# astra-vision/rain-rendering

Hardware: AMD Instinct MI355X
Metric: rainy frames/sec @ 1242x375, 100 mm/hr (higher is better)
Workload: dtype f64 alpha/mask, f32 colour

## Files before the change

__graft_entry__.py:

```python
import importlib
import os
import subprocess
import sys
import tempfile

ROOT = os.path.dirname(os.path.abspath(__file__))
if ROOT not in sys.path:
    sys.path.insert(0, ROOT)

CSRC = os.path.join(ROOT, 'rain-rendering_amd', 'csrc')
HIPCC = os.environ.get('HIPCC', '/opt/rocm/bin/hipcc')
HIP_FLAGS = ['--offload-arch=gfx950', '-O3', '-std=c++17', '-ffp-contract=off', '-fPIC', '-shared',
             '-Wno-unused-value', '-Wno-unused-result']


def _newer(target, sources):
    if not os.path.exists(target):
        return True
    t = os.path.getmtime(target)
    return any(os.path.getmtime(s) > t for s in sources)


def build(force=False):
    hip_src = os.path.join(CSRC, 'rainhip.hip')
    host_src = os.path.join(CSRC, 'rr_host.cpp')
    png_src = os.path.join(CSRC, 'rr_png.cpp')
    hip_dep = [hip_src, host_src, png_src] + sorted(os.path.join(CSRC, f) for f in os.listdir(CSRC) if f.endswith('.h')) + \
              [os.path.join(ROOT, 'include', 'rainhip.h')]
    lib = os.path.join(CSRC, 'librainhip.so')
    if force or _newer(lib, hip_dep):
        inc = ['-I' + os.path.join(ROOT, 'include'), '-I' + CSRC]
        objs = [os.path.join(CSRC, 'rainhip.o')]
        compile_flags = [f for f in HIP_FLAGS if f != '-shared']
        subprocess.check_call([HIPCC] + compile_flags + inc + ['-c', hip_src, '-o', objs[0]])
        for src in (host_src, png_src):
            obj = os.path.join(CSRC, os.path.basename(src)[:-4] + '.o')
            subprocess.check_call(['g++', '-O2', '-std=c++17', '-ffp-contract=off', '-fPIC', '-pthread', '-c'] + inc + [src, '-o', obj])
            objs.append(obj)
        subprocess.check_call([HIPCC, '--offload-arch=gfx950', '-fPIC', '-shared'] + objs + ['-lz', '-lpthread', '-o', lib])
    emu_src = os.path.join(ROOT, 'tests', 'hostemu', 'hostemu.cpp')
    emu = os.path.join(ROOT, 'tests', 'hostemu', 'libhostemu.so')
    if force or _newer(emu, [emu_src] + hip_dep[2:]):
        subprocess.check_call(['g++', '-O2', '-std=c++17', '-ffp-contract=off', '-fPIC', '-shared',
                               '-I' + os.path.join(ROOT, 'include'), '-I' + CSRC, emu_src, '-o', emu])
    noise_src = os.path.join(ROOT, 'tests', 'hostemu', 'noise_emu.cpp')
    noise_lib = os.path.join(ROOT, 'tests', 'hostemu', 'libnoiseemu.so')
    if force or _newer(noise_lib, [noise_src] + hip_dep[3:]):
        subprocess.check_call(['g++', '-O2', '-std=c++17', '-ffp-contract=off', '-fPIC', '-shared',
                               '-I' + os.path.join(ROOT, 'include'), '-I' + CSRC, noise_src, '-o', noise_lib])
    field_src = os.path.join(ROOT, 'tests', 'hostemu', 'field_emu.cpp')
    field_lib = os.path.join(ROOT, 'tests', 'hostemu', 'libfieldemu.so')
    if force or _newer(field_lib, [field_src] + hip_dep[3:]):
        subprocess.check_call(['g++', '-O2', '-std=c++17', '-ffp-contract=off', '-fPIC', '-shared',
                               '-I' + os.path.join(ROOT, 'include'), '-I' + CSRC, field_src, '-o', field_lib])
    rig_src = os.path.join(ROOT, 'tests', 'hostemu', 'rig_emu.cpp')
    rig_lib = os.path.join(ROOT, 'tests', 'hostemu', 'librigemu.so')
    if force or _newer(rig_lib, [rig_src] + hip_dep[3:]):
        subprocess.check_call(['g++', '-O2', '-std=c++17', '-ffp-contract=off', '-fPIC', '-shared',
                               '-I' + os.path.join(ROOT, 'include'), '-I' + CSRC, rig_src, '-o', rig_lib])
    importlib.import_module('rain-rendering_amd')
    hb = importlib.import_module('rain-rendering_amd.hip_backend')
    hb.load_library()


def smoke():
    import numpy as np
    build()
    sys.path.insert(0, os.path.join(ROOT, 'tests'))
    import helpers as h
    with tempfile.TemporaryDirectory() as tmp:
        sc = h.Scene(tmp, 96, 160, 120)
        bg, env = sc.frame_inputs(0)
        drops = sc.product_drops(0)
        rh = h.hb.RainHip(0)
        rh.set_streak_db(sc.db.streaks_light)
        rh.set_camera(sc.cam)
        out = rh.render_frames([dict(bg=bg, rainy_bg=bg, env_xyY=env, omega=sc.omega, drops=drops)])[0]
        ref = h.oracle_render(sc, 0, bg, bg, env, faithful=True)
        assert np.array_equal(out['status'], ref['status']), 'drop status mismatch'
        assert np.array_equal(out['mask'], ref['mask']), 'rainy_mask (f64) not bit-exact'
        assert np.array_equal(out['mask_i32'], ref['mask_i32']), 'rainy_mask (i32) not bit-exact'
        d = np.abs(out['image_u8'].astype(int) - ref['image_u8'].astype(int)).max()
        assert d <= 1, 'rainy_image differs by %d LSB' % d
        rh.close()
    print('smoke ok: %d drops, mask bit-exact, image max |d| = %d LSB' % (len(drops), d))


if __name__ == '__main__':
    build(force='--force' in sys.argv)
    if '--smoke' in sys.argv:
        smoke()
```

rain-rendering_amd/csrc/rainhip.hip:

```cpp
#include <hip/hip_runtime.h>

#include <dlfcn.h>

#include <cstddef>
#include <cstdio>
#include <cstdlib>
#include <algorithm>
#include <cstring>
#include <string>
#include <mutex>
#include <unordered_map>
#include <vector>

#include "rainhip.h"
#include "rr_device.h"
#include "rr_prepass.h"
#include "rr_deflate.h"
#include "rr_pngrows.h"
#include "rr_particles.h"

using namespace rr;

namespace {

// ... 2395 lines not shown
    }
  }
}

__global__ __launch_bounds__(1024) void k_rows_scatter(int max_drops, Scratch sc) {
  const int f = blockIdx.x, t = threadIdx.x;
  __shared__ int s_start[RW_TEX_MAX], s_rank[RW_TEX_MAX];
  const int nf = sc.rows_n[3 * f] + sc.rows_n[3 * f + 1];
  if (nf == 0) return;
  const int own = t < sc.n_buckets ? sc.rows_hist[t] : 0;
  s_start[t] = own;
  __syncthreads();
  for (int ofs = 1; ofs < 1024; ofs <<= 1) {
    const int v = t >= ofs ? s_start[t - ofs] : 0;
    __syncthreads();
    s_start[t] += v;
    __syncthreads();
  }
  const int excl = s_start[t] - own;
  __syncthreads();
  s_start[t] = excl;
  s_rank[t] = t < sc.n_buckets ? sc.rows_fbase[(int64_t)f * RW_TEX_MAX + t] : 0;
  __syncthreads();
  const int64_t base = (int64_t)f * max_drops;
  for (int j = t; j < nf; j += 1024) {
    const int i = sc.rows_list[base + j];
    const DropPlan& p = sc.plan[base + i];
    const int tex = p.tex + (p.kind == KIND_BIG ? sc.n_tex : 0);
    const int pos = s_start[tex] + atomicAdd(&s_rank[tex], 1);
    sc.rows_sorted[pos] = (int32_t)(base + i);
  }
}

__device__ void gauss_half_table(double sigma, int r, double* hw ) {
  const int t = threadIdx.x;
  for (int k = t; k <= r; k += blockDim.x) hw[k] = gauss_phi(sigma, r - k);
  __syncthreads();
  __shared__ double s_tot;
  if (t == 0) {
    double tot = 0.0;
    for (int x = -r; x <= r; x++) tot = tot + hw[r - (x < 0 ? -x : x)];
    s_tot = tot;
  }
  __syncthreads();
  const double tot = s_tot;
  for (int k = t; k <= r; k += blockDim.x) hw[k] = hw[k] / tot;
  __syncthreads();
}


constexpr int BW_LANES = 4;
__global__ __launch_bounds__(256) void k_blur_weights(const FrameDesc* frames, int max_drops, Scratch sc) {
  constexpr int NG = 256 / BW_LANES;
  __shared__ double s_hw[NG][BR_MAX + 2];
  const int f = blockIdx.y, grp = threadIdx.x / BW_LANES, l = threadIdx.x % BW_LANES;
  const int idx = blockIdx.x * NG + grp;
  const int i = idx >> 1, axis = idx & 1;
  int r = 0;
  double sigma = 0.0;
  const int64_t gi = (int64_t)f * max_drops + (i < frames[f].n_drops ? i : 0);
  if (i < frames[f].n_drops) {
    const DropPlan& p = sc.plan[gi];
    if (p.status == RR_DROP_OK && sc.sizes[gi] != 0 && p.r1 > 0 && p.r1 <= BR_MAX) {
      r = axis ? p.r2 : p.r1;
      sigma = axis ? p.sig2 : p.sig1;
    }
  }
  double* tab = s_hw[grp];
  for (int k = l; k <= r && r > 0; k += BW_LANES) tab[k] = gauss_phi(sigma, r - k);
  wave_lds_sync();
  if (l == 0 && r > 0) {
    double tot = 0.0;
    for (int x = -r; x <= r; x++) tot = tot + tab[r - (x < 0 ? -x : x)];
    tab[BR_MAX + 1] = tot;
  }
  wave_lds_sync();
  if (r > 0) {
    const double tot = tab[BR_MAX + 1];
    double* hw = sc.wtab + (gi * 2 + axis) * (BR_MAX + 1);
    for (int k = l; k <= r; k += BW_LANES) hw[k] = tab[k] / tot;
  }
}

template <class W>
__device__ inline void blur4(const double* c0, int st, W hw, int r, double& acc0, double& acc1, double& acc2, double& acc3) {
  auto at = [&](int k) { return c0[__mul24(k, st)]; };
  const double wc = hw(r);
  acc0 = c0[0] * wc; acc1 = at(1) * wc; acc2 = at(2) * wc; acc3 = at(3) * wc;
  double a0 = at(-r), a1 = at(1 - r), a2 = at(2 - r), a3 = at(3 - r);
  double b0 = at(r), b1 = at(1 + r), b2 = at(2 + r), b3 = at(3 + r);
  int ii = -r;
  for (; ii + 3 < 0; ii += 4) {
    const double w0 = hw(ii + r), w1 = hw(ii + 1 + r), w2 = hw(ii + 2 + r), w3 = hw(ii + 3 + r);
    const double na0 = at(4 + ii), na1 = at(5 + ii), na2 = at(6 + ii), na3 = at(7 + ii);
    const double nb0 = at(-ii - 1), nb1 = at(-ii - 2), nb2 = at(-ii - 3), nb3 = at(-ii - 4);
    acc0 = acc0 + (a0 + b0) * w0; acc1 = acc1 + (a1 + b1) * w0; acc2 = acc2 + (a2 + b2) * w0; acc3 = acc3 + (a3 + b3) * w0;
    acc0 = acc0 + (a1 + nb0) * w1; acc1 = acc1 + (a2 + b0) * w1; acc2 = acc2 + (a3 + b1) * w1; acc3 = acc3 + (na0 + b2) * w1;
    acc0 = acc0 + (a2 + nb1) * w2; acc1 = acc1 + (a3 + nb0) * w2; acc2 = acc2 + (na0 + b0) * w2; acc3 = acc3 + (na1 + b1) * w2;
    acc0 = acc0 + (a3 + nb2) * w3; acc1 = acc1 + (na0 + nb1) * w3; acc2 = acc2 + (na1 + nb0) * w3; acc3 = acc3 + (na2 + b0) * w3;
    a0 = na0; a1 = na1; a2 = na2; a3 = na3;
    b3 = nb0; b2 = nb1; b1 = nb2; b0 = nb3;
  }
  for (; ii < 0; ii++) {
    const double w = hw(ii + r);
    const double na = at(4 + ii);
    const double nb = at(-ii - 1);
    acc0 = acc0 + (a0 + b0) * w;
    acc1 = acc1 + (a1 + b1) * w;
    acc2 = acc2 + (a2 + b2) * w;
    acc3 = acc3 + (a3 + b3) * w;
    a0 = a1; a1 = a2; a2 = a3; a3 = na;
    b3 = b2; b2 = b1; b1 = b0; b0 = nb;
  }
}

template <int NO, class W>
__device__ inline void blur_n(const double* c0, int st, W hw, int r, double (&acc)[NO]) {
  const double wc = hw(r);
#pragma unroll
  for (int j = 0; j < NO; j++) acc[j] = c0[__mul24(j, st)] * wc;
  for (int ii = -r; ii < 0; ii++) {
    const double w = hw(ii + r);
#pragma unroll
    for (int j = 0; j < NO; j++) acc[j] = acc[j] + (c0[__mul24(j + ii, st)] + c0[__mul24(j - ii, st)]) * w;
  }
}

__device__ inline void glds_dword(const void* src, uint32_t lds_byte) {
  uint32_t keep;
  asm volatile("s_mov_b32 %0, m0\n\ts_mov_b32 m0, %2\n\ts_nop 0\n\tglobal_load_lds_dword %1, off\n\ts_mov_b32 m0, %0"
               : "=&s"(keep)
               : "v"(src), "s"(__builtin_amdgcn_readfirstlane((int)lds_byte))
               : "memory");
}
__device__ inline void glds_dwordx4(const void* src, uint32_t lds_byte) {
  uint32_t keep;
  asm volatile("s_mov_b32 %0, m0\n\ts_mov_b32 m0, %2\n\ts_nop 0\n\tglobal_load_lds_dwordx4 %1, off\n\ts_mov_b32 m0, %0"
               : "=&s"(keep)
               : "v"(src), "s"(__builtin_amdgcn_readfirstlane((int)lds_byte))
               : "memory");
}
__global__ __launch_bounds__(256, 4) void k_blur_fused_dma(const FrameDesc* frames, int max_drops, Scratch sc) {
  const int f = blockIdx.y, t = threadIdx.x, lane = t & 63, G = gridDim.x;
  const int wave = __builtin_amdgcn_readfirstlane(t >> 6);
  extern __shared__ __attribute__((aligned(16))) double s_dyn[];
  constexpr int TAB = 2 * (BR_MAX + 1);
  double* tabs = s_dyn;
  double* X = s_dyn + 2 * TAB;
  double* Y = X + sc.blur_bx;
  const uint32_t lds_tabs = (uint32_t)(uintptr_t)(__attribute__((address_space(3))) double*)tabs;
  const uint32_t lds_x = (uint32_t)(uintptr_t)(__attribute__((address_space(3))) double*)X;
  const int n_items = sc.counts[f * 8 + 2];
  if ((int)blockIdx.x >= n_items) return;
  const global_ptr<const uint32_t> items_w = as_global(reinterpret_cast<const uint32_t*>(sc.blur_items + (int64_t)f * max_drops * BLUR_ITEMS_PER_DROP));
  const DropPlan* plans = sc.plan + (int64_t)f * max_drops;
  auto load_item = [&](int item) { return items_w[(int64_t)item * 4 + (lane & 3)]; };
  auto load_plan = [&](int i) { return as_global(reinterpret_cast<const uint32_t*>(plans + i))[lane]; };
  struct PlanView {
    int r1, r2, ew, eh, tw, th, epitch, epad;
    long long a0_off, a1_off;
  };
  auto unpack = [&](uint32_t pv) {
    auto F = [&](size_t byte_off) { return (int)__builtin_amdgcn_readlane((int)pv, (int)(byte_off / 4)); };
    PlanView o;
    o.r1 = F(offsetof(DropPlan, r1)); o.r2 = F(offsetof(DropPlan, r2)); o.ew = F(offsetof(DropPlan, ew)); o.eh = F(offsetof(DropPlan, eh));
    o.tw = F(offsetof(DropPlan, tw)); o.th = F(offsetof(DropPlan, th)); o.epitch = F(offsetof(DropPlan, epitch)); o.epad = F(offsetof(DropPlan, epad));
    o.a0_off = (long long)(((unsigned long long)(unsigned)F(offsetof(DropPlan, a0_off) + 4) << 32) | (unsigned)F(offsetof(DropPlan, a0_off)));
    o.a1_off = (long long)(((unsigned long long)(unsigned)F(offsetof(DropPlan, a1_off) + 4) << 32) | (unsigned)F(offsetof(DropPlan, a1_off)));
    return o;
  };
  auto item_of = [&](uint32_t iv) {
    return make_int4((int)__builtin_amdgcn_readlane((int)iv, 0), (int)__builtin_amdgcn_readlane((int)iv, 1),
                     (int)__builtin_amdgcn_readlane((int)iv, 2), (int)__builtin_amdgcn_readlane((int)iv, 3));
  };
  struct Geo {
    int y0, x0, ho, wo, hop, hi, yp, xa, wd, nx, xs, ys, e_lo, e_hi;
  };
  auto geo = [&](const PlanView& p, int Lwo, int Lho, int st) {
    Geo g;
    const int ntx = (p.ew + Lwo - 1) / Lwo;
    const int sty = st / ntx, stx = st - sty * ntx;
    g.y0 = sty * Lho; g.x0 = stx * Lwo;
    g.ho = imin(Lho, p.eh - g.y0);
    g.wo = imin(Lwo, p.ew - g.x0);
    g.hop = (g.ho + 3) & ~3;
    const int wi = g.wo + 2 * p.r2;
    g.hi = g.hop + 2 * p.r1;
    g.yp = blur_y_pitch(g.wo, p.r2);
    g.xa = imax(0, 2 * p.r2 - g.x0);
    const int xb = imin(wi, p.tw + 2 * p.r2 - g.x0);
    g.wd = imax(xb - g.xa, 0);
    g.nx = g.wd * g.hi;
    g.xs = g.x0 - 2 * p.r2 + g.xa; g.ys = g.y0 - 2 * p.r1;
    const int ra = imin(imax(-g.ys, 0), g.hi), rb = imax(imin(p.th - g.ys, g.hi), ra);
    g.e_lo = ra * g.wd; g.e_hi = rb * g.wd;
    return g;
  };
  auto stage = [&](const PlanView& p, const Geo& g, int drop, bool tables, int tb) {
    if (g.e_hi > g.e_lo && g.wd == p.tw) {
      const char* src = reinterpret_cast<const char*>(sc.arena + p.a0_off + (int64_t)g.ys * p.tw);
      const int a = (g.e_lo + 1) & ~1, b = g.e_hi & ~1;
      for (int e0 = (a & ~511); e0 < b; e0 += 512) {
        const int e = e0 + wave * 128 + 2 * lane;
        if (e >= a && e < b) glds_dwordx4(src + (int64_t)e * 8, lds_x + (uint32_t)(e0 + wave * 128) * 8u);
      }
      if (wave == 0 && (g.e_lo & 1) && lane < 2) glds_dword(src + (int64_t)g.e_lo * 8 + lane * 4, lds_x + (uint32_t)g.e_lo * 8u);
      if (wave == 1 && (g.e_hi & 1) && g.e_hi - 1 >= g.e_lo && lane < 2) glds_dword(src + (int64_t)(g.e_hi - 1) * 8 + lane * 4, lds_x + (uint32_t)(g.e_hi - 1) * 8u);
    } else if (g.e_hi > g.e_lo) {
      const int wdd = imax(g.wd, 1);
      const float inv_wd = 1.0f / (float)wdd;
      const int dq = (int)((128.0f + 0.5f) * inv_wd), dr = 128 - dq * wdd;
      const char* src = reinterpret_cast<const char*>(sc.arena + p.a0_off) + (lane & 1) * 4;
      const int c0 = g.e_lo >> 7, c1 = (g.e_hi + 127) >> 7;
      int e = c0 * 128 + wave * 32 + (lane >> 1);
      int yy = (int)(((float)e + 0.5f) * inv_wd), xc = e - yy * wdd;
      for (int c = c0; c < c1; c++) {
        if (e >= g.e_lo && e < g.e_hi)
          glds_dword(src + (int64_t)((g.ys + yy) * p.tw + (g.xs + xc)) * 8, lds_x + (uint32_t)(c * 128 + wave * 32) * 8u);
        e += 128;
        xc += dr;
        yy += dq;
        if (xc >= wdd) { xc -= wdd; yy += 1; }
      }
    }
    if (tables) {
      const char* wt = reinterpret_cast<const char*>(sc.wtab + ((int64_t)f * max_drops + drop) * TAB);
      if (wave == 3 && lane < TAB / 2) glds_dwordx4(wt + lane * 16, lds_tabs + (uint32_t)(tb * TAB) * 8u);
    }
  };
  uint32_t iv0 = load_item(blockIdx.x);
  uint32_t pv0 = load_plan((int)__builtin_amdgcn_readlane((int)iv0, 0));
  uint32_t iv1 = load_item(imin((int)blockIdx.x + G, n_items - 1));
  uint32_t pv1 = load_plan((int)__builtin_amdgcn_readlane((int)iv1, 0));
  uint32_t iv2 = load_item(imin((int)blockIdx.x + 2 * G, n_items - 1));
  int it = blockIdx.x;
  int4 item = item_of(iv0);
  PlanView p = unpack(pv0);
  int st = item.y, tb = 0;
  Geo g = geo(p, item.w & 0xffff, item.w >> 16, st);
  stage(p, g, item.x, true, tb);
  PH_DECL
  for (;;) {
    const int r1 = p.r1, r2 = p.r2;
    const double* hw1 = tabs + tb * TAB;
    const double* hw2 = hw1 + (BR_MAX + 1);
    {
      const int nz2 = (g.yp * g.hop + 1) >> 1;
      double2* Y2 = reinterpret_cast<double2*>(Y);
      for (int i = t; i < nz2; i += 256) Y2[i] = make_double2(0.0, 0.0);
    }
    asm volatile("s_waitcnt vmcnt(0)" ::: "memory");
    bool has_next = true, new_item = false;
    int4 nitem = item;
    PlanView np = p;
    int nst = st + 1, ntb = tb;
    if (nst >= item.y + item.z) {
      if (it + G < n_items) {
        new_item = true;
        nitem = item_of(iv1);
        np = unpack(pv1);
        nst = nitem.y;
        if (nitem.x != item.x) ntb = tb ^ 1;
      } else {
        has_next = false;
      }
    }
    {
      iv1 = new_item ? iv2 : iv1;
      pv1 = load_plan((int)__builtin_amdgcn_readlane((int)iv1, 0));
      iv2 = load_item(imin(new_item ? it + 3 * G : it + 2 * G, n_items - 1));
    }
    for (int i = t; i < g.e_lo; i += 256) X[i] = 0.0;
    for (int i = g.e_hi + t; i < g.nx; i += 256) X[i] = 0.0;
    PH(0)
    __syncthreads();
    PH(1)
    {
      const int wd = g.wd, nrb = g.hop >> 2, nv = nrb * wd;
      const float inv_wd = 1.0f / (float)imax(wd, 1);
      for (int idx = t; idx < nv; idx += 256) {
        const int rb = (int)(((float)idx + 0.5f) * inv_wd), xq = idx - rb * wd;
        const double* c0 = X + (4 * rb + r1) * wd + xq;
        double acc0, acc1, acc2, acc3;
        blur4(c0, wd, [&](int k) { return hw1[k]; }, r1, acc0, acc1, acc2, acc3);
        double* o = Y + 4 * rb * g.yp + g.xa + xq;
        o[0] = acc0;
        o[g.yp] = acc1;
        o[2 * g.yp] = acc2;
        o[3 * g.yp] = acc3;
      }
    }
    PH(2)
    __syncthreads();
    PH(3)
    Geo ng = g;
    if (has_next) {
      ng = geo(np, nitem.w & 0xffff, nitem.w >> 16, nst);
      stage(np, ng, nitem.x, ntb != tb, ntb);
    }
    PH(6)
    {
      const int ncb = (g.wo + 3) >> 2, nh = ncb * g.ho;
      const float inv_ho = 1.0f / (float)g.ho;
      double* dst = sc.arena + p.a1_off;
      for (int idx = t; idx < nh; idx += 256) {
        const int cb = (int)(((float)idx + 0.5f) * inv_ho), yq = idx - cb * g.ho;
        const double* c0 = Y + yq * g.yp + 4 * cb + r2;
        double acc0, acc1, acc2, acc3;
        if (r2 > 0) {
          blur4(c0, 1, [&](int k) { return hw2[k]; }, r2, acc0, acc1, acc2, acc3);
        } else {
          acc0 = c0[0]; acc1 = c0[1]; acc2 = c0[2]; acc3 = c0[3];
        }
        const int xo = 4 * cb;
        double* o = dst + (int64_t)(g.y0 + yq) * p.epitch + p.epad + (g.x0 + xo);
        if (xo + 3 < g.wo) {
          o[0] = acc0; o[1] = acc1; o[2] = acc2; o[3] = acc3;
        } else {
          o[0] = acc0;
          if (xo + 1 < g.wo) o[1] = acc1;
          if (xo + 2 < g.wo) o[2] = acc2;
        }
      }
    }
    PH(4)
    if (!has_next) break;
    __syncthreads();
    PH(5)
    if (new_item) it += G;
    item = nitem; p = np; st = nst; tb = ntb; g = ng;
  }
  PH_FLUSH(3)
}

typedef double double2_v __attribute__((ext_vector_type(2)));
struct SmallItem {
  int li, r1, r2, tw, th, pw, ph, epitch, epad;
  long long a0, a1;
};
__global__ __launch_bounds__(256, 4) void k_blur_small(const FrameDesc* frames, int max_drops, Scratch sc) {
  const int f = blockIdx.y, lane = threadIdx.x & 63, wave = threadIdx.x >> 6;
  __shared__ __attribute__((aligned(16))) double Xs[4][BS_X], Ys[4][BS_Y];
  double* X = Xs[wave];
  double* Y = Ys[wave];
  const int n_items = sc.counts[f * 8 + 4];
  const global_ptr<const int32_t> list = as_global(sc.list_small + (int64_t)f * max_drops);
  const DropPlan* plans = sc.plan + (int64_t)f * max_drops;
  const int stride = gridDim.x * 4;
  int it = blockIdx.x * 4 + wave;
  if (it >= n_items) return;
  auto load_plan = [&](int li) { return as_global(reinterpret_cast<const uint32_t*>(plans + li))[lane]; };
  auto unpack = [&](uint32_t pv, int li) {
    auto F = [&](size_t byte_off) { return (int)__builtin_amdgcn_readlane((int)pv, (int)(byte_off / 4)); };
    static_assert(offsetof(DropPlan, a1_off) + 8 <= 256, "DropPlan layout");
    SmallItem o;
    o.li = li;
    o.r1 = F(offsetof(DropPlan, r1)); o.r2 = F(offsetof(DropPlan, r2)); o.tw = F(offsetof(DropPlan, tw)); o.th = F(offsetof(DropPlan, th));
    o.pw = F(offsetof(DropPlan, ew)); o.ph = F(offsetof(DropPlan, eh)); o.epitch = F(offsetof(DropPlan, epitch)); o.epad = F(offsetof(DropPlan, epad));
    o.a0 = (long long)(((unsigned long long)(unsigned)F(offsetof(DropPlan, a0_off) + 4) << 32) | (unsigned)F(offsetof(DropPlan, a0_off)));
    o.a1 = (long long)(((unsigned long long)(unsigned)F(offsetof(DropPlan, a1_off) + 4) << 32) | (unsigned)F(offsetof(DropPlan, a1_off)));
    return o;
  };
  double2_v R[4];
  double nw1 = 0.0, nw2 = 0.0;
  auto issue = [&](const SmallItem& d) {
    const global_ptr<const double2_v> raw2 = as_global(reinterpret_cast<const double2_v*>(sc.arena + d.a0));
    const int n = d.tw * d.th;
#pragma unroll
    for (int j = 0; j < 4; j++) {
      const int k2 = lane + 64 * j;
      R[j] = double2_v{0.0, 0.0};
      if (2 * k2 < n) R[j] = raw2[k2];
    }
    const global_ptr<const double> wt = as_global(sc.wtab + ((int64_t)f * max_drops + d.li) * 2 * (BR_MAX + 1));
    nw1 = (lane <= d.r1) ? wt[d.r1 - lane] : 0.0;
    nw2 = (d.r2 > 0 && lane <= d.r2) ? wt[(BR_MAX + 1) + d.r2 - lane] : 0.0;
  };
  PH_DECL
  const int li0 = __builtin_amdgcn_readfirstlane(list[it]);
  SmallItem cur = unpack(load_plan(li0), li0);
  issue(cur);
  bool has_next = it + stride < n_items;
  int li1 = has_next ? __builtin_amdgcn_readfirstlane(list[it + stride]) : li0;
  uint32_t pv_next = load_plan(li1);
  int32_t li2_v = (it + 2 * stride < n_items) ? list[it + 2 * stride] : 0;
  for (;;) {
    const int r1 = cur.r1, r2 = cur.r2, pw = cur.pw, ph = cur.ph, tw = cur.tw, th = cur.th;
    const int php = (ph + 3) & ~3, hi = php + 2 * r1, yp = blur_y_pitch(pw, r2);
    double* tile = sc.arena + cur.a1;
    {
      const int n = tw * th, top = 2 * r1 * tw;
      double2* X2 = reinterpret_cast<double2*>(X);
#pragma unroll
      for (int j = 0; j < 4; j++) {
        const int k2 = lane + 64 * j;
        if (2 * k2 < n) X2[(top >> 1) + k2] = make_double2(R[j].x, 2 * k2 + 1 < n ? R[j].y : 0.0);
      }
      for (int i = lane; i < (top >> 1); i += 64) X2[i] = make_double2(0.0, 0.0);
      const int e0 = (top + n + 1) >> 1, e1 = (tw * hi + 1) >> 1;
      for (int i = e0 + lane; i < e1; i += 64) X2[i] = make_double2(0.0, 0.0);
      const int nz2 = (yp * php + 1) >> 1;
      double2* Y2 = reinterpret_cast<double2*>(Y);
      for (int i = lane; i < nz2; i += 64) Y2[i] = make_double2(0.0, 0.0);
    }
    const double w1 = nw1, w2 = nw2;
    wave_lds_sync();
    PH(0)
    SmallItem nxt = cur;
    if (has_next) {
      nxt = unpack(pv_next, li1);
      issue(nxt);
      if (it + 2 * stride < n_items) {
        li1 = __builtin_amdgcn_readfirstlane(li2_v);
        pv_next = load_plan(li1);
        if (it + 3 * stride < n_items) li2_v = list[it + 3 * stride];
      }
    }
    const float inv_tw = 1.0f / (float)tw;
    const int nv4 = (php >> 2) * tw;
    if (nv4 <= 16) {
      const int idx = lane;
      if (idx < 4 * nv4) {
        const int row = (int)(((float)idx + 0.5f) * inv_tw), x = idx - row * tw;
        double a[1];
        blur_n<1>(X + (__mul24(row + r1, tw) + x), tw, [&](int k) { return readlane_f64(w1, r1 - k); }, r1, a);
        Y[__mul24(row, yp) + 2 * r2 + x] = a[0];
      }
    } else if (nv4 <= 32) {
      const int idx = lane;
      if (idx < 2 * nv4) {
        const int rb = (int)(((float)idx + 0.5f) * inv_tw), x = idx - rb * tw;
        double a[2];
        blur_n<2>(X + (__mul24(2 * rb + r1, tw) + x), tw, [&](int k) { return readlane_f64(w1, r1 - k); }, r1, a);
        double* o = Y + (__mul24(2 * rb, yp) + 2 * r2 + x);
        o[0] = a[0];
        o[yp] = a[1];
      }
    } else {
      const int nv = nv4;
      for (int idx = lane; idx < nv; idx += 64) {
        const int rb = (int)(((float)idx + 0.5f) * inv_tw), x = idx - rb * tw;
        const double* c0 = X + (__mul24(4 * rb + r1, tw) + x);
        double a0, a1, a2, a3;
        blur4(c0, tw, [&](int k) { return readlane_f64(w1, r1 - k); }, r1, a0, a1, a2, a3);
        double* o = Y + (__mul24(4 * rb, yp) + 2 * r2 + x);
        o[0] = a0;
        o[yp] = a1;
        o[2 * yp] = a2;
        o[3 * yp] = a3;
      }
    }
    wave_lds_sync();
    PH(1)
    const int ncb = (pw + 3) >> 2, nh = ncb * ph;
    const float inv_ph = 1.0f / (float)ph;
    if (nh <= 16 && r2 > 0) {
      const int idx = lane;
      if (idx < pw * ph) {
        const int x = (int)(((float)idx + 0.5f) * inv_ph), yq = idx - x * ph;
        double a[1];
        blur_n<1>(Y + (__mul24(yq, yp) + x + r2), 1, [&](int k) { return readlane_f64(w2, r2 - k); }, r2, a);
        tile[(int64_t)yq * cur.epitch + cur.epad + x] = a[0];
      }
    } else if (nh <= 32 && r2 > 0) {
      const int idx = lane, nc2 = (pw + 1) >> 1;
      if (idx < nc2 * ph) {
        const int cb = (int)(((float)idx + 0.5f) * inv_ph), yq = idx - cb * ph, xo = 2 * cb;
        double a[2];
        blur_n<2>(Y + (__mul24(yq, yp) + xo + r2), 1, [&](int k) { return readlane_f64(w2, r2 - k); }, r2, a);
        double* o = tile + (int64_t)yq * cur.epitch + cur.epad + xo;
        o[0] = a[0];
        if (xo + 1 < pw) o[1] = a[1];
      }
    } else {
      for (int idx = lane; idx < nh; idx += 64) {
        const int cb = (int)(((float)idx + 0.5f) * inv_ph), yq = idx - cb * ph;
        const double* c0 = Y + (__mul24(yq, yp) + 4 * cb + r2);
        double a0, a1, a2, a3;
        if (r2 > 0) {
          blur4(c0, 1, [&](int k) { return readlane_f64(w2, r2 - k); }, r2, a0, a1, a2, a3);
        } else {
          a0 = c0[0]; a1 = c0[1]; a2 = c0[2]; a3 = c0[3];
        }
        const int xo = 4 * cb;
        double* o = tile + (int64_t)yq * cur.epitch + cur.epad + xo;
        if (xo + 3 < pw) {
          o[0] = a0; o[1] = a1; o[2] = a2; o[3] = a3;
        } else {
          o[0] = a0;
          if (xo + 1 < pw) o[1] = a1;
          if (xo + 2 < pw) o[2] = a2;
        }
      }
    }
    wave_lds_sync();
    PH(2)
    if (!has_next) break;
    it += stride;
    cur = nxt;
    has_next = it + stride < n_items;
  }
  PH_FLUSH(2)
}

constexpr int BIG_GROUPS = 64;
constexpr int BIG_ROWS = 16;
constexpr int BIG_COL_LDS = 2048;

template <class F>
__device__ inline void visit_taps(int a0, int a1, int b0, int b1, int r, F f) {
  a0 = imax(a0, -r); a1 = imin(a1, -1);
  b0 = imax(b0, -r); b1 = imin(b1, -1);
  if (a0 > a1) { a0 = b0; a1 = b1; b0 = 0; b1 = -1; }
  if (b0 <= b1 && b0 < a0) { int t = a0; a0 = b0; b0 = t; t = a1; a1 = b1; b1 = t; }
  if (b0 <= b1 && b0 <= a1 + 1) { a1 = imax(a1, b1); b0 = 0; b1 = -1; }
  for (int ii = a0; ii <= a1; ii++) f(ii);
  for (int ii = b0; ii <= b1; ii++) f(ii);
}

constexpr int SLOW_CAP = 256;
__global__ __launch_bounds__(256) void k_blur_big_weights(const FrameDesc* frames, int max_drops, Scratch sc) {
  const int f = blockIdx.y;
  __shared__ double hw[MAX_R + 1];
  const int n_items = imin(sc.counts[f * 8 + 3], SLOW_CAP);
  for (int w = blockIdx.x; w < 2 * n_items; w += gridDim.x) {
    const int it = w >> 1, axis = w & 1;
    const DropPlan& p = sc.plan[(int64_t)f * max_drops + sc.list_slow[(int64_t)f * max_drops + it]];
    const int r = axis ? p.r2 : p.r1;
    __syncthreads();
    if (r > 0) {
      gauss_half_table(axis ? p.sig2 : p.sig1, r, hw);
      double* o = sc.wtab_big + (((int64_t)f * SLOW_CAP + it) * 2 + axis) * (MAX_R + 1);
      for (int k = threadIdx.x; k <= r; k += 256) o[k] = hw[k];
    }
  }
}

template <int AXIS>
__global__ __launch_bounds__(256) void k_blur(const FrameDesc* frames, int max_drops, Scratch sc) {
  const int f = blockIdx.y, t = threadIdx.x;
  __shared__ double hw[MAX_R + 1];
  __shared__ double s_in[BIG_COL_LDS];
  const int n_items = sc.counts[f * 8 + 3];
  int cur = -1;
  for (int w = blockIdx.x; w < n_items * BIG_GROUPS; w += gridDim.x) {
    const int it = w / BIG_GROUPS, g = w - it * BIG_GROUPS;
    const int64_t gi = (int64_t)f * max_drops + sc.list_slow[(int64_t)f * max_drops + it];
    const DropPlan& p = sc.plan[gi];
    const int r = AXIS == 0 ? p.r1 : p.r2;
    const int tw = p.tw, th = p.th, ew = p.ew, eh = p.eh, r1 = p.r1, r2 = p.r2;
    if (AXIS == 0 ? g >= tw : g * BIG_ROWS >= eh) continue;
    const double* raw = sc.arena + p.a0_off;
    double* fin = sc.arena + p.a1_off;
    double* tmp = fin + (((int64_t)p.epitch * eh + 15) & ~15LL);
    __syncthreads();
    if (cur != it) {
      if (r > 0) {
        if (it < SLOW_CAP) {
          const double* wt = sc.wtab_big + (((int64_t)f * SLOW_CAP + it) * 2 + AXIS) * (MAX_R + 1);
          for (int k = t; k <= r; k += 256) hw[k] = wt[k];
          __syncthreads();
        } else {
          gauss_half_table(AXIS == 0 ? p.sig1 : p.sig2, r, hw);
        }
      }
      cur = it;
    }
    if (AXIS == 0) {
      for (int rx = g; rx < tw; rx += BIG_GROUPS) {
        const bool lds = th <= BIG_COL_LDS;
        __syncthreads();
        if (lds)
          for (int k = t; k < th; k += 256) s_in[k] = raw[(int64_t)k * tw + rx];
        __syncthreads();
// ... 4182 lines not shown
```

rain-rendering_amd/csrc/rr_device.h:

```cpp
#pragma once
#include <math.h>
#include <stdint.h>

#include "rainhip.h"

#if defined(__HIPCC__)
#include <hip/hip_runtime.h>
#define RR_HD __host__ __device__ inline
#else
#define RR_HD inline
#endif

#if defined(__clang__)
#pragma clang fp contract(off)
#endif

namespace rr {

enum { KIND_BIG = 0, KIND_ROT = 1, KIND_EXT = 2 };
enum { RS_AREA = 0, RS_AREA_FAST = 1, RS_LINEAR = 2 };

struct Dims {
  int32_t H, W, He, We;
};
// ... 1230 lines not shown
      else p.rs_mode = RS_AREA;
    } else {
      p.rs_mode = RS_LINEAR;
    }
    minCx = d.x0;
    minCy = d.y0;
  }

  if (strategy == 1) {
    p.pw = p.tw;
    p.ph = p.th;
    const int sx = py_slice_index(minCx, W), ex = py_slice_index(minCx + p.tw, W);
    const int sy = py_slice_index(minCy, H), ey = py_slice_index(minCy + p.th, H);
    p.vis_x0 = sx;
    p.vis_y0 = sy;
    p.vis_w = imax(ex - sx, 0);
    p.vis_h = imax(ey - sy, 0);
    p.tau_one = cam.exposure_s * 1.0;
    p.g = p.tau_one / cam.tau_zero;
    p.ew = p.tw;
    p.eh = p.th;
    size_out = (p.vis_w > 0 && p.vis_h > 0) ? (((int64_t)p.tw * p.th + 15) & ~15LL) : 0;
    return;
  }
  double o = fabs(d.wps[2]);
  double cc = ((o - cam.focus_plane) * cam.focal_sq) / (o * (cam.focus_plane - cam.focal_m) * cam.f_number);
  cc = fabs(cc / cam.sensor_px);
  if (!(cc < 1.7e308)) { p.status = RR_DROP_BAD_COC; return; }
  if (10.0 * cc >= (double)(RR_MAX_SHIFT + 1)) { p.status = RR_DROP_TOO_BIG; return; }
  p.shift = (int)(10.0 * cc);
  p.sig1 = cc;
  p.sig2 = cc / 2.0;
  p.r1 = (p.sig1 > 1e-15) ? (int)(4.0 * p.sig1 + 0.5) : 0;
  p.r2 = (p.sig2 > 1e-15) ? (int)(4.0 * p.sig2 + 0.5) : 0;
  p.pw = p.tw + 2 * p.shift;
  p.ph = p.th + 2 * p.shift;

  int tmpx = minCx - p.shift, tmpy = minCy - p.shift;
  int mcx = imin(imax(tmpx, 0), W), mcy = imin(imax(tmpy, 0), H);
  int dx = mcx - tmpx, dy = mcy - tmpy;
  int cw, ch;
  if (dx < 0) { cw = imax(p.pw + dx, 0); p.crop_x = 0; } else { cw = imax(p.pw - dx, 0); p.crop_x = dx; }
  if (dy < 0) { ch = imax(p.ph + dy, 0); p.crop_y = 0; } else { ch = imax(p.ph - dy, 0); p.crop_y = dy; }
  p.vis_x0 = mcx;
  p.vis_y0 = mcy;
  p.vis_w = imax(imin(mcx + cw, W) - mcx, 0);
  p.vis_h = imax(imin(mcy + ch, H) - mcy, 0);

  double d_avg = (d.iw1 + d.iw2) / 2.0;
  double length_opacity = opacity_attenuation * d_avg / ((double)d.length + d_avg);
  p.tau_one = cam.exposure_s * length_opacity;
  p.g = p.tau_one / cam.tau_zero;

  p.ew = p.tw + 2 * p.r2;
  p.eh = p.th + 2 * p.r1;
  p.epad = 0;
  p.epitch = p.ew;
  size_out = (p.vis_w > 0 && p.vis_h > 0) ? (((int64_t)p.tw * p.th + 15) & ~15LL) + (p.r1 > 0 ? (((int64_t)p.epitch * p.eh + 15) & ~15LL) : 0) : 0;
}

RR_HD double blur_axis0(const double* src, int pw, int ph, int x, int y, const double* hw, int r) {
  double acc = src[(int64_t)y * pw + x] * hw[r];
  for (int ii = -r; ii < 0; ii++) {
    int ya = y + ii, yb = y - ii;
    double va = (ya >= 0) ? src[(int64_t)ya * pw + x] : 0.0;
    double vb = (yb < ph) ? src[(int64_t)yb * pw + x] : 0.0;
    acc = acc + (va + vb) * hw[ii + r];
  }
  return acc;
}
RR_HD double blur_axis1(const double* src, int pw, int ph, int x, int y, const double* hw, int r) {
  (void)ph;
  const double* row = src + (int64_t)y * pw;
  double acc = row[x] * hw[r];
  for (int ii = -r; ii < 0; ii++) {
    int xa = x + ii, xb = x - ii;
    double va = (xa >= 0) ? row[xa] : 0.0;
    double vb = (xb < pw) ? row[xb] : 0.0;
    acc = acc + (va + vb) * hw[ii + r];
  }
  return acc;
}

RR_HD void blend_pixel(double A, double tau_one, double exposure, double g, const double K[3], double bgr[3], double& mask) {
  double t = (A * tau_one) / exposure;
  double u = 1.0 - t;
  for (int c = 0; c < 3; c++) {
    double v = u * bgr[c] + (A * K[c]) * g;
    bgr[c] = clip01(v);
  }
  mask = mask + A;
}

constexpr int BLUR_BX = 2816;
constexpr int BLUR_BY = 2048;
constexpr int BR_MAX = 48;

struct BlurLayout {
  int fused;
  int wo, ho;
  int single;
};
RR_HD int blur_x_doubles(int wo, int ho, int r1, int r2, int tw) { return imin(wo + 2 * r2, tw) * (((ho + 3) & ~3) + 2 * r1); }
RR_HD int blur_y_pitch(int wo, int r2) { return (((wo + 3) & ~3) + 2 * r2) | 1; }
RR_HD int blur_y_doubles(int wo, int ho, int r2) { return blur_y_pitch(wo, r2) * ((ho + 3) & ~3); }

RR_HD BlurLayout blur_layout(const DropPlan& p, int BX_MAX, int BY_MAX) {
  BlurLayout b{0, 0, 0, 0};
  if (p.r1 <= 0 || p.r1 > BR_MAX) return b;
  if (blur_x_doubles(p.ew, p.eh, p.r1, p.r2, p.tw) <= BX_MAX && blur_y_doubles(p.ew, p.eh, p.r2) <= BY_MAX) {
    b.fused = 1; b.wo = p.ew; b.ho = p.eh; b.single = 1;
    return b;
  }
  {
    const int hy = (BY_MAX / blur_y_pitch(p.ew, p.r2)) & ~3;
    const int hx = ((BX_MAX / imin(p.ew + 2 * p.r2, p.tw)) - 2 * p.r1) & ~3;
    const int hb = imin(hy, hx);
    if (hb >= imax(8, p.r1)) {
      b.fused = 1; b.wo = p.ew; b.ho = imin(hb, p.eh);
      return b;
    }
  }
  const double rr2 = (double)imax(p.r2, 1), rr1 = (double)p.r1;
  int wi = (int)sqrt((double)BX_MAX * rr2 / rr1);
  wi = imax(imin(wi, p.ew + 2 * p.r2), 2 * p.r2 + 4);
  int hi = BX_MAX / wi;
  hi = imin(hi, ((p.eh + 3) & ~3) + 2 * p.r1);
  wi = imin(BX_MAX / hi, p.ew + 2 * p.r2);
  int wo = wi - 2 * p.r2, ho = (hi - 2 * p.r1) & ~3;
  if (ho > p.eh) ho = p.eh;
  for (int it = 0; it < 64 && wo >= 1 && ho >= 1; it++) {
    if (blur_x_doubles(wo, ho, p.r1, p.r2, p.tw) <= BX_MAX && blur_y_doubles(wo, ho, p.r2) <= BY_MAX) {
      b.fused = 1; b.wo = wo; b.ho = ho; b.single = (wo >= p.ew && ho >= p.eh) ? 1 : 0;
      return b;
    }
    if (blur_x_doubles(wo, ho, p.r1, p.r2, p.tw) > BX_MAX) { if (wo > 4) wo -= 1; else ho -= 4; }
    else ho -= 4;
  }
  return b;
}
constexpr int BS_X = 512;
constexpr int BS_Y = 768;

RR_HD bool blur_is_small(const DropPlan& p) {
  const int php = (p.eh + 3) & ~3;
  return p.r1 > 0 && p.r1 <= 31 && p.tw * (php + 2 * p.r1) <= BS_X && blur_y_pitch(p.ew, p.r2) * php <= BS_Y;
}


}
```

Measured before the change: 18440.

## Blur eight outputs per thread with a generic sliding-window kernel

Replaces the hand-unrolled 4-output separable blur with a templated sliding-window routine. Larger tiles now process 8 rows or columns per thread, with a 4-wide tail, so each loaded sample is reused across more outputs. The per-item Y buffer clear now zeroes only the padding columns instead of the whole buffer. The change also adds readfirstlane hints for wave-uniform offsets and the wave index, plus a host emulator build for the blur. Register pressure rises with 8 accumulators under launch_bounds(256,4), and any mismatch in the reassociated summation order would break the required bit-exact masks.

```diff
diff --git a/__graft_entry__.py b/__graft_entry__.py
--- a/__graft_entry__.py
+++ b/__graft_entry__.py
@@ -58,6 +58,11 @@
     if force or _newer(rig_lib, [rig_src] + hip_dep[3:]):
         subprocess.check_call(['g++', '-O2', '-std=c++17', '-ffp-contract=off', '-fPIC', '-shared',
                                '-I' + os.path.join(ROOT, 'include'), '-I' + CSRC, rig_src, '-o', rig_lib])
+    blur_src = os.path.join(ROOT, 'tests', 'hostemu', 'blur_emu.cpp')
+    blur_lib = os.path.join(ROOT, 'tests', 'hostemu', 'libbluremu.so')
+    if force or _newer(blur_lib, [blur_src] + hip_dep[3:]):
+        subprocess.check_call(['g++', '-O2', '-std=c++17', '-ffp-contract=off', '-fPIC', '-shared',
+                               '-I' + os.path.join(ROOT, 'include'), '-I' + CSRC, blur_src, '-o', blur_lib])
     importlib.import_module('rain-rendering_amd')
     hb = importlib.import_module('rain-rendering_amd.hip_backend')
     hb.load_library()
diff --git a/rain-rendering_amd/csrc/rainhip.hip b/rain-rendering_amd/csrc/rainhip.hip
--- a/rain-rendering_amd/csrc/rainhip.hip
+++ b/rain-rendering_amd/csrc/rainhip.hip
@@ -2501,49 +2501,6 @@
   }
 }
 
-template <class W>
-__device__ inline void blur4(const double* c0, int st, W hw, int r, double& acc0, double& acc1, double& acc2, double& acc3) {
-  auto at = [&](int k) { return c0[__mul24(k, st)]; };
-  const double wc = hw(r);
-  acc0 = c0[0] * wc; acc1 = at(1) * wc; acc2 = at(2) * wc; acc3 = at(3) * wc;
-  double a0 = at(-r), a1 = at(1 - r), a2 = at(2 - r), a3 = at(3 - r);
-  double b0 = at(r), b1 = at(1 + r), b2 = at(2 + r), b3 = at(3 + r);
-  int ii = -r;
-  for (; ii + 3 < 0; ii += 4) {
-    const double w0 = hw(ii + r), w1 = hw(ii + 1 + r), w2 = hw(ii + 2 + r), w3 = hw(ii + 3 + r);
-    const double na0 = at(4 + ii), na1 = at(5 + ii), na2 = at(6 + ii), na3 = at(7 + ii);
-    const double nb0 = at(-ii - 1), nb1 = at(-ii - 2), nb2 = at(-ii - 3), nb3 = at(-ii - 4);
-    acc0 = acc0 + (a0 + b0) * w0; acc1 = acc1 + (a1 + b1) * w0; acc2 = acc2 + (a2 + b2) * w0; acc3 = acc3 + (a3 + b3) * w0;
-    acc0 = acc0 + (a1 + nb0) * w1; acc1 = acc1 + (a2 + b0) * w1; acc2 = acc2 + (a3 + b1) * w1; acc3 = acc3 + (na0 + b2) * w1;
-    acc0 = acc0 + (a2 + nb1) * w2; acc1 = acc1 + (a3 + nb0) * w2; acc2 = acc2 + (na0 + b0) * w2; acc3 = acc3 + (na1 + b1) * w2;
-    acc0 = acc0 + (a3 + nb2) * w3; acc1 = acc1 + (na0 + nb1) * w3; acc2 = acc2 + (na1 + nb0) * w3; acc3 = acc3 + (na2 + b0) * w3;
-    a0 = na0; a1 = na1; a2 = na2; a3 = na3;
-    b3 = nb0; b2 = nb1; b1 = nb2; b0 = nb3;
-  }
-  for (; ii < 0; ii++) {
-    const double w = hw(ii + r);
-    const double na = at(4 + ii);
-    const double nb = at(-ii - 1);
-    acc0 = acc0 + (a0 + b0) * w;
-    acc1 = acc1 + (a1 + b1) * w;
-    acc2 = acc2 + (a2 + b2) * w;
-    acc3 = acc3 + (a3 + b3) * w;
-    a0 = a1; a1 = a2; a2 = a3; a3 = na;
-    b3 = b2; b2 = b1; b1 = b0; b0 = nb;
-  }
-}
-
-template <int NO, class W>
-__device__ inline void blur_n(const double* c0, int st, W hw, int r, double (&acc)[NO]) {
-  const double wc = hw(r);
-#pragma unroll
-  for (int j = 0; j < NO; j++) acc[j] = c0[__mul24(j, st)] * wc;
-  for (int ii = -r; ii < 0; ii++) {
-    const double w = hw(ii + r);
-#pragma unroll
-    for (int j = 0; j < NO; j++) acc[j] = acc[j] + (c0[__mul24(j + ii, st)] + c0[__mul24(j - ii, st)]) * w;
-  }
-}
 
 __device__ inline void glds_dword(const void* src, uint32_t lds_byte) {
   uint32_t keep;
@@ -2695,18 +2652,35 @@
     __syncthreads();
     PH(1)
     {
-      const int wd = g.wd, nrb = g.hop >> 2, nv = nrb * wd;
+      const int wd = g.wd, nv4 = (g.hop >> 2) * wd;
       const float inv_wd = 1.0f / (float)imax(wd, 1);
-      for (int idx = t; idx < nv; idx += 256) {
-        const int rb = (int)(((float)idx + 0.5f) * inv_wd), xq = idx - rb * wd;
-        const double* c0 = X + (4 * rb + r1) * wd + xq;
-        double acc0, acc1, acc2, acc3;
-        blur4(c0, wd, [&](int k) { return hw1[k]; }, r1, acc0, acc1, acc2, acc3);
-        double* o = Y + 4 * rb * g.yp + g.xa + xq;
-        o[0] = acc0;
-        o[g.yp] = acc1;
-        o[2 * g.yp] = acc2;
-        o[3 * g.yp] = acc3;
+      auto w1 = [&](int k) { return hw1[k]; };
+      auto rows4 = [&](int row, int xq) {
+        double acc[4];
+        blur4(X + (row + r1) * wd + xq, wd, w1, r1, acc);
+        double* o = Y + row * g.yp + g.xa + xq;
+#pragma unroll
+        for (int j = 0; j < 4; j++) o[__mul24(j, g.yp)] = acc[j];
+      };
+      if (nv4 > 256) {
+        const int n8 = (g.hop >> 3) * wd, n4 = (g.hop & 4) ? wd : 0;
+        for (int idx = t; idx < n8 + n4; idx += 256) {
+          if (idx < n8) {
+            const int rb = (int)(((float)idx + 0.5f) * inv_wd), xq = idx - rb * wd;
+            double acc[8];
+            blur8(X + (8 * rb + r1) * wd + xq, wd, w1, r1, acc);
+            double* o = Y + 8 * rb * g.yp + g.xa + xq;
+#pragma unroll
+            for (int j = 0; j < 8; j++) o[__mul24(j, g.yp)] = acc[j];
+          } else {
+            rows4(g.hop & ~7, idx - n8);
+          }
+        }
+      } else {
+        for (int idx = t; idx < nv4; idx += 256) {
+          const int rb = (int)(((float)idx + 0.5f) * inv_wd);
+          rows4(4 * rb, idx - rb * wd);
+        }
       }
     }
     PH(2)
@@ -2719,26 +2693,58 @@
     }
     PH(6)
     {
-      const int ncb = (g.wo + 3) >> 2, nh = ncb * g.ho;
+      const int wop = (g.wo + 3) & ~3, nh4 = (wop >> 2) * g.ho;
       const float inv_ho = 1.0f / (float)g.ho;
       double* dst = sc.arena + p.a1_off;
-      for (int idx = t; idx < nh; idx += 256) {
-        const int cb = (int)(((float)idx + 0.5f) * inv_ho), yq = idx - cb * g.ho;
-        const double* c0 = Y + yq * g.yp + 4 * cb + r2;
-        double acc0, acc1, acc2, acc3;
+      auto w2 = [&](int k) { return hw2[k]; };
+      auto cols4 = [&](int yq, int xo) {
+        const double* c0 = Y + yq * g.yp + xo + r2;
+        double acc[4];
         if (r2 > 0) {
-          blur4(c0, 1, [&](int k) { return hw2[k]; }, r2, acc0, acc1, acc2, acc3);
+          blur4(c0, 1, w2, r2, acc);
         } else {
-          acc0 = c0[0]; acc1 = c0[1]; acc2 = c0[2]; acc3 = c0[3];
+#pragma unroll
+          for (int j = 0; j < 4; j++) acc[j] = c0[j];
         }
-        const int xo = 4 * cb;
         double* o = dst + (int64_t)(g.y0 + yq) * p.epitch + p.epad + (g.x0 + xo);
         if (xo + 3 < g.wo) {
-          o[0] = acc0; o[1] = acc1; o[2] = acc2; o[3] = acc3;
+          o[0] = acc[0]; o[1] = acc[1]; o[2] = acc[2]; o[3] = acc[3];
         } else {
-          o[0] = acc0;
-          if (xo + 1 < g.wo) o[1] = acc1;
-          if (xo + 2 < g.wo) o[2] = acc2;
+          o[0] = acc[0];
+          if (xo + 1 < g.wo) o[1] = acc[1];
+          if (xo + 2 < g.wo) o[2] = acc[2];
+        }
+      };
+      if (nh4 > 256) {
+        const int n8 = (wop >> 3) * g.ho, n4 = (wop & 4) ? g.ho : 0;
+        for (int idx = t; idx < n8 + n4; idx += 256) {
+          if (idx < n8) {
+            const int cb = (int)(((float)idx + 0.5f) * inv_ho), yq = idx - cb * g.ho, xo = 8 * cb;
+            const double* c0 = Y + yq * g.yp + xo + r2;
+            double acc[8];
+            if (r2 > 0) {
+              blur8(c0, 1, w2, r2, acc);
+            } else {
+#pragma unroll
+              for (int j = 0; j < 8; j++) acc[j] = c0[j];
+            }
+            double* o = dst + (int64_t)(g.y0 + yq) * p.epitch + p.epad + (g.x0 + xo);
+            if (xo + 7 < g.wo) {
+#pragma unroll
+              for (int j = 0; j < 8; j++) o[j] = acc[j];
+            } else {
+#pragma unroll
+              for (int j = 0; j < 8; j++)
+                if (xo + j < g.wo) o[j] = acc[j];
+            }
+          } else {
+            cols4(idx - n8, wop & ~7);
+          }
+        }
+      } else {
+        for (int idx = t; idx < nh4; idx += 256) {
+          const int cb = (int)(((float)idx + 0.5f) * inv_ho);
+          cols4(idx - cb * g.ho, 4 * cb);
         }
       }
     }
@@ -2758,7 +2764,7 @@
   long long a0, a1;
 };
 __global__ __launch_bounds__(256, 4) void k_blur_small(const FrameDesc* frames, int max_drops, Scratch sc) {
-  const int f = blockIdx.y, lane = threadIdx.x & 63, wave = threadIdx.x >> 6;
+  const int f = blockIdx.y, lane = threadIdx.x & 63, wave = __builtin_amdgcn_readfirstlane(threadIdx.x >> 6);
   __shared__ __attribute__((aligned(16))) double Xs[4][BS_X], Ys[4][BS_Y];
   double* X = Xs[wave];
   double* Y = Ys[wave];
@@ -2802,10 +2808,11 @@
   bool has_next = it + stride < n_items;
   int li1 = has_next ? __builtin_amdgcn_readfirstlane(list[it + stride]) : li0;
   uint32_t pv_next = load_plan(li1);
-  int32_t li2_v = (it + 2 * stride < n_items) ? list[it + 2 * stride] : 0;
+  auto list_ahead = [&](int i) { asm("" : "+v"(i)); return list[i]; };
+  int32_t li2_v = (it + 2 * stride < n_items) ? list_ahead(it + 2 * stride) : 0;
   for (;;) {
     const int r1 = cur.r1, r2 = cur.r2, pw = cur.pw, ph = cur.ph, tw = cur.tw, th = cur.th;
-    const int php = (ph + 3) & ~3, hi = php + 2 * r1, yp = blur_y_pitch(pw, r2);
+    const int php = (ph + 3) & ~3, hi = php + 2 * r1, yp = blur_y_pitch(pw, r2), pwp = (pw + 3) & ~3;
     double* tile = sc.arena + cur.a1;
     {
       const int n = tw * th, top = 2 * r1 * tw;
@@ -2818,9 +2825,12 @@
       for (int i = lane; i < (top >> 1); i += 64) X2[i] = make_double2(0.0, 0.0);
       const int e0 = (top + n + 1) >> 1, e1 = (tw * hi + 1) >> 1;
       for (int i = e0 + lane; i < e1; i += 64) X2[i] = make_double2(0.0, 0.0);
-      const int nz2 = (yp * php + 1) >> 1;
-      double2* Y2 = reinterpret_cast<double2*>(Y);
-      for (int i = lane; i < nz2; i += 64) Y2[i] = make_double2(0.0, 0.0);
+      const int nl = 2 * r2, nzc = nl + pwp - tw, nz = __mul24(ph, nzc);
+      const float inv_nzc = 1.0f / (float)imax(nzc, 1);
+      for (int i = lane; i < nz; i += 64) {
+        const int row = (int)(((float)i + 0.5f) * inv_nzc), k = i - __mul24(row, nzc);
+        Y[__mul24(row, yp) + (k < nl ? k : k + tw)] = 0.0;
+      }
     }
     const double w1 = nw1, w2 = nw2;
     wave_lds_sync();
@@ -2832,17 +2842,19 @@
       if (it + 2 * stride < n_items) {
         li1 = __builtin_amdgcn_readfirstlane(li2_v);
         pv_next = load_plan(li1);
-        if (it + 3 * stride < n_items) li2_v = list[it + 3 * stride];
+        if (it + 3 * stride < n_items) li2_v = list_ahead(it + 3 * stride);
       }
     }
     const float inv_tw = 1.0f / (float)tw;
+    auto hw1 = [&](int k) { return readlane_f64(w1, r1 - k); };
+    auto hw2 = [&](int k) { return readlane_f64(w2, r2 - k); };
     const int nv4 = (php >> 2) * tw;
     if (nv4 <= 16) {
       const int idx = lane;
       if (idx < 4 * nv4) {
         const int row = (int)(((float)idx + 0.5f) * inv_tw), x = idx - row * tw;
         double a[1];
-        blur_n<1>(X + (__mul24(row + r1, tw) + x), tw, [&](int k) { return readlane_f64(w1, r1 - k); }, r1, a);
+        blur_n<1>(X + (__mul24(row + r1, tw) + x), tw, hw1, r1, a);
         Y[__mul24(row, yp) + 2 * r2 + x] = a[0];
       }
     } else if (nv4 <= 32) {
@@ -2850,35 +2862,50 @@
       if (idx < 2 * nv4) {
         const int rb = (int)(((float)idx + 0.5f) * inv_tw), x = idx - rb * tw;
         double a[2];
-        blur_n<2>(X + (__mul24(2 * rb + r1, tw) + x), tw, [&](int k) { return readlane_f64(w1, r1 - k); }, r1, a);
+        blur_n<2>(X + (__mul24(2 * rb + r1, tw) + x), tw, hw1, r1, a);
         double* o = Y + (__mul24(2 * rb, yp) + 2 * r2 + x);
         o[0] = a[0];
         o[yp] = a[1];
       }
     } else {
-      const int nv = nv4;
-      for (int idx = lane; idx < nv; idx += 64) {
-        const int rb = (int)(((float)idx + 0.5f) * inv_tw), x = idx - rb * tw;
-        const double* c0 = X + (__mul24(4 * rb + r1, tw) + x);
-        double a0, a1, a2, a3;
-        blur4(c0, tw, [&](int k) { return readlane_f64(w1, r1 - k); }, r1, a0, a1, a2, a3);
-        double* o = Y + (__mul24(4 * rb, yp) + 2 * r2 + x);
-        o[0] = a0;
-        o[yp] = a1;
-        o[2 * yp] = a2;
-        o[3 * yp] = a3;
+      auto rows4 = [&](int row, int x) {
+        double a[4];
+        blur4(X + (__mul24(row + r1, tw) + x), tw, hw1, r1, a);
+        double* o = Y + (__mul24(row, yp) + 2 * r2 + x);
+#pragma unroll
+        for (int j = 0; j < 4; j++) o[__mul24(j, yp)] = a[j];
+      };
+      if (nv4 > 64) {
+        const int n8 = (php >> 3) * tw, n4 = (php & 4) ? tw : 0;
+        for (int idx = lane; idx < n8 + n4; idx += 64) {
+          if (idx < n8) {
+            const int rb = (int)(((float)idx + 0.5f) * inv_tw), x = idx - rb * tw;
+            double a[8];
+            blur8(X + (__mul24(8 * rb + r1, tw) + x), tw, hw1, r1, a);
+            double* o = Y + (__mul24(8 * rb, yp) + 2 * r2 + x);
+#pragma unroll
+            for (int j = 0; j < 8; j++) o[__mul24(j, yp)] = a[j];
+          } else {
+            rows4(php & ~7, idx - n8);
+          }
+        }
+      } else {
+        for (int idx = lane; idx < nv4; idx += 64) {
+          const int rb = (int)(((float)idx + 0.5f) * inv_tw);
+          rows4(4 * rb, idx - rb * tw);
+        }
       }
     }
     wave_lds_sync();
     PH(1)
-    const int ncb = (pw + 3) >> 2, nh = ncb * ph;
+    const int nh = (pwp >> 2) * ph;
     const float inv_ph = 1.0f / (float)ph;
     if (nh <= 16 && r2 > 0) {
       const int idx = lane;
       if (idx < pw * ph) {
         const int x = (int)(((float)idx + 0.5f) * inv_ph), yq = idx - x * ph;
         double a[1];
-        blur_n<1>(Y + (__mul24(yq, yp) + x + r2), 1, [&](int k) { return readlane_f64(w2, r2 - k); }, r2, a);
+        blur_n<1>(Y + (__mul24(yq, yp) + x + r2), 1, hw2, r2, a);
         tile[(int64_t)yq * cur.epitch + cur.epad + x] = a[0];
       }
     } else if (nh <= 32 && r2 > 0) {
@@ -2886,29 +2913,60 @@
       if (idx < nc2 * ph) {
         const int cb = (int)(((float)idx + 0.5f) * inv_ph), yq = idx - cb * ph, xo = 2 * cb;
         double a[2];
-        blur_n<2>(Y + (__mul24(yq, yp) + xo + r2), 1, [&](int k) { return readlane_f64(w2, r2 - k); }, r2, a);
+        blur_n<2>(Y + (__mul24(yq, yp) + xo + r2), 1, hw2, r2, a);
         double* o = tile + (int64_t)yq * cur.epitch + cur.epad + xo;
         o[0] = a[0];
         if (xo + 1 < pw) o[1] = a[1];
       }
     } else {
-      for (int idx = lane; idx < nh; idx += 64) {
-        const int cb = (int)(((float)idx + 0.5f) * inv_ph), yq = idx - cb * ph;
-        const double* c0 = Y + (__mul24(yq, yp) + 4 * cb + r2);
-        double a0, a1, a2, a3;
+      auto cols4 = [&](int yq, int xo) {
+        const double* c0 = Y + (__mul24(yq, yp) + xo + r2);
+        double a[4];
         if (r2 > 0) {
-          blur4(c0, 1, [&](int k) { return readlane_f64(w2, r2 - k); }, r2, a0, a1, a2, a3);
+          blur4(c0, 1, hw2, r2, a);
         } else {
-          a0 = c0[0]; a1 = c0[1]; a2 = c0[2]; a3 = c0[3];
+#pragma unroll
+          for (int j = 0; j < 4; j++) a[j] = c0[j];
         }
-        const int xo = 4 * cb;
         double* o = tile + (int64_t)yq * cur.epitch + cur.epad + xo;
         if (xo + 3 < pw) {
-          o[0] = a0; o[1] = a1; o[2] = a2; o[3] = a3;
+          o[0] = a[0]; o[1] = a[1]; o[2] = a[2]; o[3] = a[3];
         } else {
-          o[0] = a0;
-          if (xo + 1 < pw) o[1] = a1;
-          if (xo + 2 < pw) o[2] = a2;
+          o[0] = a[0];
+          if (xo + 1 < pw) o[1] = a[1];
+          if (xo + 2 < pw) o[2] = a[2];
+        }
+      };
+      if (nh > 64) {
+        const int n8 = (pwp >> 3) * ph, n4 = (pwp & 4) ? ph : 0;
+        for (int idx = lane; idx < n8 + n4; idx += 64) {
+          if (idx < n8) {
+            const int cb = (int)(((float)idx + 0.5f) * inv_ph), yq = idx - cb * ph, xo = 8 * cb;
+            const double* c0 = Y + (__mul24(yq, yp) + xo + r2);
+            double a[8];
+            if (r2 > 0) {
+              blur8(c0, 1, hw2, r2, a);
+            } else {
+#pragma unroll
+              for (int j = 0; j < 8; j++) a[j] = c0[j];
+            }
+            double* o = tile + (int64_t)yq * cur.epitch + cur.epad + xo;
+            if (xo + 7 < pw) {
+#pragma unroll
+              for (int j = 0; j < 8; j++) o[j] = a[j];
+            } else {
+#pragma unroll
+              for (int j = 0; j < 8; j++)
+                if (xo + j < pw) o[j] = a[j];
+            }
+          } else {
+            cols4(idx - n8, pwp & ~7);
+          }
+        }
+      } else {
+        for (int idx = lane; idx < nh; idx += 64) {
+          const int cb = (int)(((float)idx + 0.5f) * inv_ph);
+          cols4(idx - cb * ph, 4 * cb);
         }
       }
     }
diff --git a/rain-rendering_amd/csrc/rr_device.h b/rain-rendering_amd/csrc/rr_device.h
--- a/rain-rendering_amd/csrc/rr_device.h
+++ b/rain-rendering_amd/csrc/rr_device.h
@@ -1336,6 +1336,65 @@
   return acc;
 }
 
+RR_HD int blur_running_offset(int o) {
+#if defined(__HIP_DEVICE_COMPILE__)
+#if defined(RR_DEBUG_UNIFORM)
+  if (__builtin_amdgcn_readfirstlane(o) != o) __builtin_trap();
+#endif
+  o = __builtin_amdgcn_readfirstlane(o);
+#endif
+  return o;
+}
+template <int N, class W>
+RR_HD void blur_window(const double* c0, int st, W hw, int r, double (&acc)[N]) {
+  double a[N], b[N];
+  const double wc = hw(r);
+  int oa = mul24i(-r, st), ob = mul24i(r, st);
+#pragma unroll
+  for (int j = 0; j < N; j++) {
+    acc[j] = c0[j * st] * wc;
+    a[j] = c0[oa + j * st];
+    b[j] = c0[ob + j * st];
+  }
+  oa += N * st;
+  ob -= st;
+  double w = hw(0);
+  for (int ii = -r; ii < 0; ii += N) {
+    oa = blur_running_offset(oa);
+    ob = blur_running_offset(ob);
+#pragma unroll
+    for (int s = 0; s < N; s++) {
+      if (s > 0 && ii + s >= 0) return;
+      const double na = c0[oa + s * st], nb = c0[ob - s * st];
+      const double wn = hw(ii + s + 1 + r);
+#pragma unroll
+      for (int j = 0; j < N; j++) acc[j] = acc[j] + (a[(j + s) % N] + b[(j - s + N) % N]) * w;
+      a[s] = na;
+      b[N - 1 - s] = nb;
+      w = wn;
+    }
+    oa += N * st;
+    ob -= N * st;
+  }
+}
+template <class W>
+RR_HD void blur4(const double* c0, int st, W hw, int r, double (&acc)[4]) { blur_window<4>(c0, st, hw, r, acc); }
+template <class W>
+RR_HD void blur8(const double* c0, int st, W hw, int r, double (&acc)[8]) { blur_window<8>(c0, st, hw, r, acc); }
+
+template <int NO, class W>
+RR_HD void blur_n(const double* c0, int st, W hw, int r, double (&acc)[NO]) {
+  const double wc = hw(r);
+#pragma unroll
+  for (int j = 0; j < NO; j++) acc[j] = c0[j * st] * wc;
+  int oa = mul24i(-r, st), ob = mul24i(r, st);
+  for (int ii = -r; ii < 0; ii++, oa += st, ob -= st) {
+    const double w = hw(ii + r);
+#pragma unroll
+    for (int j = 0; j < NO; j++) acc[j] = acc[j] + (c0[oa + j * st] + c0[ob + j * st]) * w;
+  }
+}
+
 RR_HD void blend_pixel(double A, double tau_one, double exposure, double g, const double K[3], double bgr[3], double& mask) {
   double t = (A * tau_one) / exposure;
   double u = 1.0 - t;
```

After: 18770 (median of 6 runs). 1.8% higher.
